# victorca25/traiNNer

Measured on AMD Instinct MI355X. Metric: HR images/sec (G+D step), ESRGAN x4 128->512, higher is better.
Workload: dtype f32 (bf16x3)

## Files before the change

include/trainner_hip.h:

```cpp
#ifndef TRAINNER_HIP_H
#define TRAINNER_HIP_H

#include <stdint.h>

#ifdef __cplusplus
extern "C" {
#endif

#define TNR_OK 0
#define TNR_EINVAL (-1)
#define TNR_ELAUNCH (-2)

enum { TNR_ACT_NONE = 0, TNR_ACT_LRELU = 1, TNR_ACT_RELU = 2 };

enum {
    TNR_CONV_3x3 = 0,
    TNR_CONV_3x3_UP2 = 1,
    TNR_CONV_4x4_S2 = 2,
    TNR_DGRAD_4x4_S2 = 3,
    TNR_CONV_1x1 = 4,
    TNR_CONV_3x3_C4 = 5,
    TNR_CONV_7x7_C4 = 6
};

// ... 13 lines not shown
#define TNR_MMA_BF16X3 2

typedef struct tnr_view {
    float *ptr;
    int32_t ctot;
    int32_t coff;
} tnr_view;

typedef struct tnr_conv_desc {
    tnr_view x;
    int32_t N, H, W;
    int32_t Cin;
    const float *wp;
    int32_t KinP, KoutP;
    tnr_view y;
    int32_t Ho, Wo, Cout;
    int32_t mode;
    const float *bias;
    int32_t act;
    float slope;
    float alpha;
    tnr_view r1; int32_t r1_ch; float beta1;
    tnr_view r2; float alpha2;
    tnr_view m;  int32_t m_lo, m_hi; float m_slope;
    float *ws; int64_t ws_bytes;
    int32_t mma;
    int32_t pad_mode;
    float noise_sigma; int32_t noise_pos; uint32_t noise_key0, noise_key1, noise_pix0;
    const void *wq; int64_t wq_bytes;
    int32_t wq_form;
    int32_t shuffle;
} tnr_conv_desc;

typedef struct tnr_wgrad_desc {
    tnr_view x; int32_t N, H, W; int32_t Cin;
    tnr_view g; int32_t Ho, Wo; int32_t Cout;
    int32_t mode;
    float *dw; int32_t cin_total, cin_begin;
    float *db;
    float alpha, beta;
    float *ws; int64_t ws_bytes;
    int32_t mma;
    int32_t pad_mode;
    float *dw2; int32_t cout_split, cin_total2;
    float *db2;
} tnr_wgrad_desc;

typedef struct tnr_pack_item {
    const float *w;
    float *wp;
    int32_t Cout, Cin, kh, kw;
    int32_t kind;
    int32_t KoutP, KinP;
    int64_t n_out;
} tnr_pack_item;

typedef struct tnr_dense_pack_item {
    const float *w[5];
    float *wp;
    int32_t nf, gc;
    int32_t t;
    int32_t KoutP, KinP;
    float scale5;
    int64_t n_out;
} tnr_dense_pack_item;

const char *tnr_last_error(void);
#define TNR_ABI_VERSION 3
int tnr_version(void);

int tnr_pack_dims(int32_t Cout, int32_t Cin, int32_t kh, int32_t kw, int32_t kind,
                  int32_t *KoutP, int32_t *KinP, int64_t *n_out);
int tnr_pack_weights(const tnr_pack_item *items_dev, int32_t n, int64_t max_out, void *stream);
int tnr_pack_dense_dims(int32_t nf, int32_t gc, int32_t t, int32_t *KoutP, int32_t *KinP, int64_t *n_out);
int tnr_pack_dense_dgrad(const tnr_dense_pack_item *items_dev, int32_t n, int64_t max_out, void *stream);
int tnr_conv_forward(const tnr_conv_desc *d, void *stream);
int tnr_gauss_mult(tnr_view dst, tnr_view src, int64_t pixels, int32_t C, float sigma, uint32_t key0, uint32_t key1, uint32_t pix0,
                   void *stream);
int64_t tnr_conv_workspace_bytes(const tnr_conv_desc *d);
int64_t tnr_conv_wq_bytes(const tnr_conv_desc *d);
int tnr_conv_wq_pack(const tnr_conv_desc *d, void *image, int64_t image_bytes, void *stream);
int64_t tnr_conv_wino_bytes(const tnr_conv_desc *d);
int tnr_conv_wino_pack(const tnr_conv_desc *d, void *image, int64_t image_bytes, void *stream);
int tnr_im2col(tnr_view x, int32_t N, int32_t H, int32_t W, int32_t C, int32_t k, int32_t stride, int32_t pad,
               int32_t Ho, int32_t Wo, float *out, void *stream);
#define TNR_CHAIN_MAX 6
int64_t tnr_conv_chain_workspace_bytes(const tnr_conv_desc *stage0);
int tnr_conv_chain(const tnr_conv_desc *stages, const int32_t *fresh_from, int32_t n, uint32_t *ws, int64_t ws_bytes,
                   uint32_t epoch, void *stream);
int64_t tnr_conv_sweep_image_bytes(const tnr_conv_desc *stages, int32_t n);
int tnr_conv_sweep_pack(const tnr_conv_desc *stages, int32_t n, void *image, int64_t image_bytes, void *stream);
typedef struct tnr_sweep_pack_item { int32_t units; int32_t reserved; uint64_t opaque[15]; } tnr_sweep_pack_item;
int tnr_conv_sweep_pack_item(const tnr_conv_desc *stages, int32_t n, void *image, int64_t image_bytes, tnr_sweep_pack_item *item);
int tnr_conv_sweep_pack_batch(const tnr_sweep_pack_item *items_dev, int32_t n, int32_t max_units, void *stream);
int tnr_conv_sweep(const tnr_conv_desc *stages, int32_t n, const void *image, uint32_t *ws, int64_t ws_bytes, uint32_t epoch,
                   void *stream);
int64_t tnr_conv_thin_pack_floats(int32_t reduce_channels);
int tnr_conv_thin_pack(const float *w_oihw, float *wp, int32_t Cout, int32_t Cin, int32_t dgrad, void *stream);
int tnr_conv_thin(tnr_view x, int32_t N, int32_t H, int32_t W, int32_t Cin, const float *wp, tnr_view y, int32_t Cout,
                  const float *bias, float alpha, void *stream);
int64_t tnr_conv_thin7_pack_floats(int32_t reduce_channels);
int tnr_conv_thin7_pack(const float *w_oihw, float *wp, int32_t Cout, int32_t Cin, int32_t dgrad, void *stream);
int tnr_conv_thin7(tnr_view x, int32_t N, int32_t H, int32_t W, int32_t Cin, const float *wp, tnr_view y, int32_t Ho, int32_t Wo,
                   int32_t Cout, int32_t pad, int32_t reflect, const float *bias, float alpha, void *stream);
int64_t tnr_wgrad_workspace_bytes(const tnr_wgrad_desc *d);
int64_t tnr_wgrad_thin_workspace_bytes(int32_t N, int32_t H, int32_t Cbig);
int tnr_wgrad_thin(tnr_view big, tnr_view small, int32_t N, int32_t H, int32_t W, int32_t Cbig, int32_t Csmall, int32_t flip,
                   float *dw, float *db, float alpha, float beta, float *ws, int64_t ws_bytes, void *stream);
int64_t tnr_wgrad_thin7_workspace_bytes(int32_t N, int32_t Hbig_grid, int32_t Cbig);
int tnr_wgrad_thin7(tnr_view big, int32_t N, int32_t H, int32_t W, int32_t rpad, tnr_view small, int32_t Hs, int32_t Ws, int32_t off,
                    int32_t Cbig, int32_t Csmall, int32_t flip, float *dw, float *db, float alpha, float beta, float *ws, int64_t ws_bytes,
                    void *stream);
int tnr_conv_wgrad(const tnr_wgrad_desc *d, void *stream);
#define TNR_WGRAD_GROUP_MAX 12
int tnr_conv_wgrad_group(const tnr_wgrad_desc *descs, int32_t n, void *stream);
int tnr_wgrad_tile_class(const tnr_wgrad_desc *d, int32_t group_jobs, int32_t x3_occ, int32_t out[12]);

int tnr_gconv_fwd(tnr_view x, int32_t N, int32_t H, int32_t W, int32_t Cin, const float *w, const float *bias, tnr_view y, int32_t Ho,
                  int32_t Wo, int32_t Cout, int32_t k, int32_t stride, int32_t pad, int32_t reflect, int32_t act, float slope, void *stream);
int tnr_gconv_dgrad(tnr_view g, int32_t N, int32_t H, int32_t W, int32_t Cin, const float *w, tnr_view gx, int32_t Ho, int32_t Wo,
                    int32_t Cout, int32_t k, int32_t stride, int32_t pad, int32_t reflect, void *stream);
int64_t tnr_gconv_wgrad_workspace_bytes(int32_t Cout, int32_t Cin, int32_t k);
int tnr_gconv_wgrad(tnr_view x, int32_t N, int32_t H, int32_t W, int32_t Cin, tnr_view g, int32_t Ho, int32_t Wo, int32_t Cout, int32_t k,
                    int32_t stride, int32_t pad, int32_t reflect, float *dw, float *db, float alpha, float beta, double *ws,
                    int64_t ws_bytes, void *stream);
int tnr_bias_grad(tnr_view g, int64_t pixels, int32_t C, float *db, float alpha, float beta, double *ws, int64_t ws_bytes, void *stream);
int tnr_pad2d(tnr_view x, tnr_view y, int32_t N, int32_t H, int32_t W, int32_t C, int32_t pad, int32_t mode, void *stream);
int tnr_unpad2d(tnr_view xp, tnr_view y, int32_t N, int32_t H, int32_t W, int32_t C, int32_t pad, int32_t mode, void *stream);
int tnr_window2d(tnr_view src, int32_t Hs, int32_t Ws, tnr_view dst, int32_t N, int32_t Hd, int32_t Wd, int32_t C, int32_t oy,
                 int32_t ox, int32_t acc, void *stream);
int tnr_tanh_fwd(const float *x, float *y, int64_t n, void *stream);
int tnr_tanh_bwd(const float *g, const float *y, float *gx, int64_t n, void *stream);
int tnr_gan_loss(const float *pred, int64_t n, int32_t type, float target, float *out, float *grad, void *stream);
int tnr_dp_unique_id(void *id128);
int tnr_dp_init(const void *id128, int32_t rank, int32_t world, void **comm);
int tnr_dp_allreduce_bucket(void *comm, float *buf, int64_t count, int32_t average, void *stream);
int tnr_dp_broadcast(void *comm, float *buf, int64_t count, int32_t root, void *stream);
int tnr_dp_comm_count(void *comm, int32_t *nranks);
int tnr_dp_finalize(void *comm);
int tnr_filter2d(const float *src, float *dst, const float *kernels21, int32_t N, int32_t C, int32_t H, int32_t W, void *stream);
int tnr_resize(const float *src, float *dst, int32_t NC, int32_t H, int32_t W, int32_t Ho, int32_t Wo, int32_t mode, void *stream);
int tnr_noise_gaussian(float *img, int32_t N, int32_t C, int32_t H, int32_t W, const float *sigma255, const int32_t *grey,
                       uint64_t seed, int32_t clip, void *stream);
int tnr_noise_poisson(float *img, int32_t N, int32_t C, int32_t H, int32_t W, const float *vals, const float *scale,
                      const int32_t *grey, uint64_t seed, int32_t clip, void *stream);
int64_t tnr_jpeg_workspace_bytes(int32_t N, int32_t H, int32_t W);
int tnr_jpeg_sim(float *img, int32_t N, int32_t H, int32_t W, const int32_t *quality, float *ws, int64_t ws_bytes, void *stream);
int tnr_feed_u8_to_tensor(const uint8_t *src, int32_t N, int32_t H, int32_t W, int32_t C, const int32_t *flags, int32_t any_rot,
                          float *dst, int32_t bgr2rgb, float data_range, int32_t normalize, void *stream);
int tnr_tensor2np_u8(const float *src, int32_t N, int32_t C, int32_t H, int32_t W, uint8_t *dst, int32_t rgb2bgr,
                     int32_t denormalize, void *stream);
int64_t tnr_metrics_workspace_bytes(int32_t N);
int tnr_psnr_ssim_u8(const uint8_t *a, const uint8_t *b, int32_t N, int32_t H, int32_t W, int32_t C, int32_t crop,
                     int32_t want_ssim, double *out, double *ws, int64_t ws_bytes, void *stream);
int tnr_lpips_stem_dims(int32_t H, int32_t W, int32_t crop, int32_t *Ho, int32_t *Wo);
int tnr_lpips_stem(const void *a, const void *b, int32_t src_kind, int32_t N, int32_t H, int32_t W, int32_t C, int32_t crop,
                   int32_t normalize, const float *shift, const float *scale, const float *w, const float *bias, tnr_view y,
                   void *stream);
int tnr_maxpool3s2_ceil_dims(int32_t H, int32_t W, int32_t *Ho, int32_t *Wo);
int tnr_maxpool3s2_ceil_fwd(tnr_view x, tnr_view y, int32_t N, int32_t H, int32_t W, int32_t C, void *stream);
int64_t tnr_lpips_workspace_bytes(int32_t N, int32_t L);
int tnr_lpips_head(tnr_view f0, tnr_view f1, int32_t N, int32_t H, int32_t W, int32_t C, const float *w, int32_t layer, int32_t L,
                   double *ws, int64_t ws_bytes, void *stream);
int tnr_lpips_finalize(int32_t N, int32_t L, const double *ws, int64_t ws_bytes, double *out, double *per_layer, void *stream);
int tnr_bilinear2x_fwd(tnr_view x, tnr_view y, int32_t N, int32_t H, int32_t W, int32_t C, void *stream);
int tnr_bilinear2x_bwd(tnr_view gy, tnr_view gx, tnr_view gz, tnr_view mask, float mslope, int32_t N, int32_t H, int32_t W,
// ... 151 lines not shown
```

trainner_amd/csrc/conv_wino.hip:

```cpp
#include <stddef.h>
#include <stdlib.h>
#include <type_traits>
#include <utility>
#include "conv_body.h"
#include "conv_epilogue.h"

namespace {

constexpr int WN_T = 16;
constexpr int WN_PT = WN_T / 2;
constexpr int WN_NP = WN_PT * WN_PT;
constexpr int WN_RAW_W = WN_T + 2;
constexpr int WN_RAW_PIX = WN_RAW_W * WN_RAW_W;
constexpr int WN_RAW_STRIDE = 24;
constexpr int WN_RAW_FLOATS = WN_RAW_PIX * WN_RAW_STRIDE;
constexpr int WN_ROW = TNR_X3_ROW;
constexpr int WN_VH_ROWS = 8 * WN_NP;
constexpr int WN_VH_FLOATS = WN_VH_ROWS * WN_ROW;
constexpr size_t WN_LDS_BYTES = (size_t)(2 * WN_VH_FLOATS + 2 * WN_RAW_FLOATS) * sizeof(float);
constexpr int WN_UNIT_FLOATS = 32 * WN_ROW;
constexpr int WN_STAGE_ITEMS = WN_RAW_PIX * 4;
constexpr int WN_STAGE_IT = (WN_STAGE_ITEMS / 2 + 255) / 256;
static_assert(WN_LDS_BYTES <= 160 * 1024, "one Winograd workgroup per CU");
static_assert(8 * 4 * 16 * 64 * sizeof(float) <= WN_LDS_BYTES, "the inverse transform's exchange fits the LDS");
// ... 523 lines not shown

        __syncthreads();
        raw_load(0, true);
        raw_store(0);
        raw_load(16, c.nck > 1);
        if (c.nck > 1) raw_store(1);
        __syncthreads();
        if (wh == 1) __syncthreads();
#pragma unroll 1
        for (int ck = 0; ck < c.nck; ++ck) {
            if (ck >= 1 && ck + 1 < c.nck) raw_store((ck + 1) & 1);
            transform(ck & 1);
            b_fetch(ck);
            __syncthreads();
            raw_load(16 * (ck + 2), ck + 2 < c.nck);
            multiply();
            __syncthreads();
        }
        if (wh == 0) __syncthreads();

        f32x16 pr_[2][2];
#pragma unroll
        for (int m = 0; m < 2; ++m) {
            if (wjp == 0) {
                pr_[0][m] = acc[0][m] + acc[1][m];
                pr_[1][m] = acc[1][m];
            } else {
                pr_[0][m] = acc[0][m];
                pr_[1][m] = -acc[0][m] - acc[1][m];
            }
        }
        float *xa = smem + (((wave & 3) | (wh << 2)) * 4) * (16 * 64);
        if (wjp == 1) {
#pragma unroll
            for (int l = 0; l < 2; ++l)
#pragma unroll
                for (int m = 0; m < 2; ++m)
#pragma unroll
                    for (int r = 0; r < 16; ++r) xa[((l * 2 + m) * 16 + r) * 64 + lane] = pr_[l][m][r];
        }
        __syncthreads();
        if (wjp == 0) {
#pragma unroll
            for (int l = 0; l < 2; ++l)
#pragma unroll
                for (int m = 0; m < 2; ++m)
#pragma unroll
                    for (int r = 0; r < 16; ++r) pr_[l][m][r] = l == 0 ? pr_[l][m][r] + xa[((l * 2 + m) * 16 + r) * 64 + lane]
                                                                       : pr_[l][m][r] + xa[((l * 2 + m) * 16 + r) * 64 + lane];
        }
        __syncthreads();
        float *xb = smem + ((wh * 4 + wn * 2 + wil) * 4) * (16 * 64);
        if (wjp == 0) {
#pragma unroll
            for (int l = 0; l < 2; ++l)
#pragma unroll
                for (int m = 0; m < 2; ++m)
#pragma unroll
                    for (int r = 0; r < 16; ++r) xb[((l * 2 + m) * 16 + r) * 64 + lane] = pr_[l][m][r];
        }
        __syncthreads();
        f32x16 keep[1][1];
        {
            const int k = wil, m = wh, l = wjp;
            auto slot = [&](int ip) __attribute__((always_inline)) {
                return smem + (((ip >> 1) * 4 + wn * 2 + (ip & 1)) * 4 + l * 2 + m) * (16 * 64) + lane;
            };
            const float *p0 = slot(k), *p1 = slot(k + 1), *p2 = slot(k + 2);
#pragma unroll
            for (int r = 0; r < 16; ++r) {
                const float x0 = p0[r * 64], x1 = p1[r * 64], x2 = p2[r * 64];
                keep[0][0][r] = k == 0 ? (x0 + x1) + x2 : (x0 - x1) - x2;
            }
        }
        conv_epilogue_dpp_map<TNR_CONV_3x3, WN_T, 1, 1, false, 1>(a, keep, cb * 2 + wn, n, ty0, tx0, 0, li, half, y_rs,
                                                                  [&](int, int row, int &rr, int &cc) __attribute__((always_inline)) {
                                                                      const int p = 32 * wh + row;
                                                                      rr = 2 * (p >> 3) + wil;
                                                                      cc = 2 * (p & 7) + wjp;
                                                                  });
    }
}

bool wino_ok(const tnr_conv_desc *d) {
    return d->mode == TNR_CONV_3x3 && d->mma == TNR_MMA_BF16X3 && (d->pad_mode == 0 || (d->pad_mode == 1 && d->H >= 2 && d->W >= 2)) &&
           (d->Cout % 64) == 0 && d->KoutP == d->Cout && d->Cin == d->KinP && (d->Cin % 16) == 0 && d->Cin >= 32 && d->Ho == d->H &&
           d->Wo == d->W && d->W >= 8 && d->H >= 8 && buffers_addressable(*d) &&
           (int64_t)(d->Cout / 64) * (d->Cin / 16) * 32 * WN_UNIT_FLOATS * (int64_t)sizeof(float) < (1LL << 31);
}

}

#ifdef WN_TIMELINE
extern "C" int tnr_debug_wino_timeline(unsigned long long *out16, int reset) {
    if (out16 != nullptr && hipMemcpyFromSymbol(out16, HIP_SYMBOL(wn_tl), sizeof(wn_tl)) != hipSuccess) return TNR_ELAUNCH;
    if (reset) {
        unsigned long long z[32] = {0};
        if (hipMemcpyToSymbol(HIP_SYMBOL(wn_tl), z, sizeof(z)) != hipSuccess) return TNR_ELAUNCH;
    }
    return TNR_OK;
}
#endif

extern "C" int64_t tnr_conv_wino_bytes(const tnr_conv_desc *d) {
    if (d == nullptr || !wino_ok(d)) return 0;
    return (int64_t)(d->Cout / 64) * (d->Cin / 16) * 32 * WN_UNIT_FLOATS * (int64_t)sizeof(float);
}

extern "C" int tnr_conv_wino_pack(const tnr_conv_desc *d, void *image, int64_t image_bytes, void *stream) {
    TNR_REQUIRE(d != nullptr && image != nullptr && d->wp != nullptr && wino_ok(d), "conv_wino_pack: the launch cannot run in the Winograd form");
    WinoPackK a;
    a.wp = d->wp; a.KinP = d->KinP; a.KoutP = d->KoutP; a.nck = d->Cin / 16; a.ncb = d->Cout / 64;
    a.units = a.ncb * a.nck * 32;
    TNR_REQUIRE((int64_t)a.units * WN_UNIT_FLOATS * (int64_t)sizeof(float) <= image_bytes, "conv_wino_pack: image buffer too small");
    a.out = static_cast<float *>(image);
    hipLaunchKernelGGL(wino_pack_kernel, dim3((unsigned)tnr_cdiv(a.units * 64, 256)), dim3(256), 0, (hipStream_t)stream, a);
    return tnr_check_launch("conv_wino_pack");
}

int tnr_launch_conv3x3_wino(const tnr_conv_desc *d, void *stream) {
    if (!wino_ok(d) || d->wq == nullptr || d->wq_bytes < tnr_conv_wino_bytes(d) || d->noise_pos < 0 || d->noise_pos > 2) return 1;
    static int cus = 0;
    if (const int rc = tnr_kernel_setup(&cus, "conv3x3_wino", {{conv3x3_wino_kernel, WN_LDS_BYTES}, {conv3x3_wino16_kernel, WN_LDS_BYTES}})) return rc;
    WinoK c;
    if (!stream_k_from_desc(c, *d, tnr_conv_wino_bytes(d), WN_T, WN_T, 1)) return 1;
    const int grid = c.tiles < cus ? c.tiles : cus;
    static const bool w16 = [] { const char *e = getenv("TNR_WINO_WAVES"); return e != nullptr && atoi(e) == 16; }();
    if (w16) {
        hipLaunchKernelGGL(conv3x3_wino16_kernel, dim3((unsigned)grid), dim3(1024), WN_LDS_BYTES, (hipStream_t)stream, c);
        return tnr_check_launch("conv3x3_wino16");
    }
    hipLaunchKernelGGL(conv3x3_wino_kernel, dim3((unsigned)grid), dim3(512), WN_LDS_BYTES, (hipStream_t)stream, c);
    return tnr_check_launch("conv3x3_wino");
}
```

trainner_amd/hip.py:

```python
import ctypes as C
import os

import torch

from . import build as _build

c_f = C.c_float
c_i = C.c_int32
c_l = C.c_int64
c_p = C.c_void_p

ACT_NONE, ACT_LRELU, ACT_RELU = 0, 1, 2
MMA_F32, MMA_BF16, MMA_BF16X3 = 0, 1, 2
CONV_3x3, CONV_3x3_UP2, CONV_4x4_S2, DGRAD_4x4_S2, CONV_1x1, CONV_3x3_C4, CONV_7x7_C4 = 0, 1, 2, 3, 4, 5, 6
PACK_FWD, PACK_DGRAD_3x3, PACK_FWD_S2D, PACK_DGRAD_S2, PACK_COL_FWD, PACK_COL_DGRAD3 = 0, 1, 2, 3, 4, 5
PACK_C4_FWD, PACK_C4_DGRAD3 = 6, 7
PACK_DENSE_DGRAD = 16


class CView(C.Structure):
    _fields_ = [("ptr", c_p), ("ctot", c_i), ("coff", c_i)]


class ConvDesc(C.Structure):
    _fields_ = [
        ("x", CView), ("N", c_i), ("H", c_i), ("W", c_i), ("Cin", c_i),
        ("wp", c_p), ("KinP", c_i), ("KoutP", c_i),
        ("y", CView), ("Ho", c_i), ("Wo", c_i), ("Cout", c_i),
        ("mode", c_i), ("bias", c_p), ("act", c_i), ("slope", c_f), ("alpha", c_f),
        ("r1", CView), ("r1_ch", c_i), ("beta1", c_f),
        ("r2", CView), ("alpha2", c_f),
        ("m", CView), ("m_lo", c_i), ("m_hi", c_i), ("m_slope", c_f),
        ("ws", c_p), ("ws_bytes", c_l), ("mma", c_i), ("pad_mode", c_i),
        ("noise_sigma", c_f), ("noise_pos", c_i), ("noise_key0", C.c_uint32), ("noise_key1", C.c_uint32), ("noise_pix0", C.c_uint32),
        ("wq", c_p), ("wq_bytes", c_l), ("wq_form", c_i), ("shuffle", c_i),
    ]


class WgradDesc(C.Structure):
    _fields_ = [
        ("x", CView), ("N", c_i), ("H", c_i), ("W", c_i), ("Cin", c_i),
        ("g", CView), ("Ho", c_i), ("Wo", c_i), ("Cout", c_i),
        ("mode", c_i),
        ("dw", c_p), ("cin_total", c_i), ("cin_begin", c_i),
        ("db", c_p), ("alpha", c_f), ("beta", c_f),
        ("ws", c_p), ("ws_bytes", c_l), ("mma", c_i), ("pad_mode", c_i),
        ("dw2", c_p), ("cout_split", c_i), ("cin_total2", c_i), ("db2", c_p),
    ]


class SweepPackItem(C.Structure):
    _fields_ = [("units", c_i), ("reserved", c_i), ("opaque", C.c_uint64 * 15)]


class PackItem(C.Structure):
    _fields_ = [("w", c_p), ("wp", c_p), ("Cout", c_i), ("Cin", c_i), ("kh", c_i), ("kw", c_i),
                ("kind", c_i), ("KoutP", c_i), ("KinP", c_i), ("n_out", c_l)]


class DensePackItem(C.Structure):
    _fields_ = [("w", c_p * 5), ("wp", c_p), ("nf", c_i), ("gc", c_i), ("t", c_i), ("KoutP", c_i), ("KinP", c_i),
                ("scale5", c_f), ("n_out", c_l)]


_SIGS = {
    "tnr_last_error": (C.c_char_p, []),
    "tnr_version": (c_i, []),
    "tnr_pack_dims": (c_i, [c_i, c_i, c_i, c_i, c_i, C.POINTER(c_i), C.POINTER(c_i), C.POINTER(c_l)]),
    "tnr_pack_weights": (c_i, [c_p, c_i, c_l, c_p]),
    "tnr_pack_dense_dims": (c_i, [c_i, c_i, c_i, C.POINTER(c_i), C.POINTER(c_i), C.POINTER(c_l)]),
    "tnr_pack_dense_dgrad": (c_i, [c_p, c_i, c_l, c_p]),
    "tnr_conv_forward": (c_i, [C.POINTER(ConvDesc), c_p]),
    "tnr_conv_workspace_bytes": (c_l, [C.POINTER(ConvDesc)]),
    "tnr_conv_wq_bytes": (c_l, [C.POINTER(ConvDesc)]),
    "tnr_conv_wq_pack": (c_i, [C.POINTER(ConvDesc), c_p, c_l, c_p]),
    "tnr_conv_wino_bytes": (c_l, [C.POINTER(ConvDesc)]),
    "tnr_conv_wino_pack": (c_i, [C.POINTER(ConvDesc), c_p, c_l, c_p]),
    "tnr_gauss_mult": (c_i, [CView, CView, c_l, c_i, c_f, C.c_uint32, C.c_uint32, C.c_uint32, c_p]),
    "tnr_im2col": (c_i, [CView, c_i, c_i, c_i, c_i, c_i, c_i, c_i, c_i, c_i, c_p, c_p]),
    "tnr_conv_chain_workspace_bytes": (c_l, [C.POINTER(ConvDesc)]),
    "tnr_conv_chain": (c_i, [C.POINTER(ConvDesc), C.POINTER(C.c_int32), c_i, c_p, c_l, C.c_uint32, c_p]),
    "tnr_conv_sweep_image_bytes": (c_l, [C.POINTER(ConvDesc), c_i]),
    "tnr_conv_sweep_pack_item": (c_i, [C.POINTER(ConvDesc), c_i, c_p, c_l, C.POINTER(SweepPackItem)]),
    "tnr_conv_sweep_pack_batch": (c_i, [c_p, c_i, c_i, c_p]),
    "tnr_conv_sweep_pack": (c_i, [C.POINTER(ConvDesc), c_i, c_p, c_l, c_p]),
    "tnr_conv_sweep": (c_i, [C.POINTER(ConvDesc), c_i, c_p, c_p, c_l, C.c_uint32, c_p]),
    "tnr_conv_thin_pack_floats": (c_l, [c_i]),
    "tnr_conv_thin_pack": (c_i, [c_p, c_p, c_i, c_i, c_i, c_p]),
    "tnr_conv_thin": (c_i, [CView, c_i, c_i, c_i, c_i, c_p, CView, c_i, c_p, c_f, c_p]),
    "tnr_wgrad_workspace_bytes": (c_l, [C.POINTER(WgradDesc)]),
    "tnr_conv_thin7_pack_floats": (c_l, [c_i]),
    "tnr_conv_thin7_pack": (c_i, [c_p, c_p, c_i, c_i, c_i, c_p]),
    "tnr_conv_thin7": (c_i, [CView, c_i, c_i, c_i, c_i, c_p, CView, c_i, c_i, c_i, c_i, c_i, c_p, c_f, c_p]),
    "tnr_wgrad_thin7_workspace_bytes": (c_l, [c_i, c_i, c_i]),
    "tnr_wgrad_thin7": (c_i, [CView, c_i, c_i, c_i, c_i, CView, c_i, c_i, c_i, c_i, c_i, c_i, c_p, c_p, c_f, c_f, c_p, c_l, c_p]),
    "tnr_wgrad_thin_workspace_bytes": (c_l, [c_i, c_i, c_i]),
    "tnr_wgrad_thin": (c_i, [CView, CView, c_i, c_i, c_i, c_i, c_i, c_i, c_p, c_p, c_f, c_f, c_p, c_l, c_p]),
    "tnr_conv_wgrad": (c_i, [C.POINTER(WgradDesc), c_p]),
    "tnr_conv_wgrad_group": (c_i, [C.POINTER(WgradDesc), c_i, c_p]),
    "tnr_wgrad_tile_class": (c_i, [C.POINTER(WgradDesc), c_i, c_i, C.POINTER(c_i * 12)]),
    "tnr_nchw_to_nhwc": (c_i, [c_p, c_i, c_i, c_i, c_i, CView, c_i, c_p, c_p, c_p]),
    "tnr_nhwc_to_nchw": (c_i, [CView, c_i, c_i, c_i, c_i, c_p, c_p, c_i, c_p]),
    "tnr_upsample2x_bwd": (c_i, [CView, CView, c_i, c_i, c_i, c_i, CView, c_f, c_p]),
    "tnr_depth_to_space": (c_i, [CView, CView, c_i, c_i, c_i, c_i, c_p]),
    "tnr_space_to_depth_bwd": (c_i, [CView, CView, c_i, c_i, c_i, c_i, CView, c_f, c_p]),
    "tnr_maxpool2_fwd": (c_i, [CView, CView, c_i, c_i, c_i, c_i, c_p]),
    "tnr_maxpool2_bwd": (c_i, [CView, CView, CView, c_i, c_i, c_i, c_i, c_p]),
    "tnr_gconv_fwd": (c_i, [CView, c_i, c_i, c_i, c_i, c_p, c_p, CView, c_i, c_i, c_i, c_i, c_i, c_i, c_i, c_i, c_f, c_p]),
    "tnr_gconv_dgrad": (c_i, [CView, c_i, c_i, c_i, c_i, c_p, CView, c_i, c_i, c_i, c_i, c_i, c_i, c_i, c_p]),
    "tnr_gconv_wgrad_workspace_bytes": (c_l, [c_i, c_i, c_i]),
    "tnr_gconv_wgrad": (c_i, [CView, c_i, c_i, c_i, c_i, CView, c_i, c_i, c_i, c_i, c_i, c_i, c_i, c_p, c_p, c_f, c_f, c_p, c_l, c_p]),
    "tnr_bias_grad": (c_i, [CView, c_l, c_i, c_p, c_f, c_f, c_p, c_l, c_p]),
    "tnr_pad2d": (c_i, [CView, CView, c_i, c_i, c_i, c_i, c_i, c_i, c_p]),
    "tnr_unpad2d": (c_i, [CView, CView, c_i, c_i, c_i, c_i, c_i, c_i, c_p]),
    "tnr_window2d": (c_i, [CView, c_i, c_i, CView, c_i, c_i, c_i, c_i, c_i, c_i, c_i, c_p]),
    "tnr_tanh_fwd": (c_i, [c_p, c_p, c_l, c_p]),
    "tnr_tanh_bwd": (c_i, [c_p, c_p, c_p, c_l, c_p]),
    "tnr_gan_loss": (c_i, [c_p, c_l, c_i, c_f, c_p, c_p, c_p]),
    "tnr_dp_unique_id": (c_i, [c_p]),
    "tnr_dp_init": (c_i, [c_p, c_i, c_i, C.POINTER(c_p)]),
    "tnr_dp_allreduce_bucket": (c_i, [c_p, c_p, c_l, c_i, c_p]),
    "tnr_dp_broadcast": (c_i, [c_p, c_p, c_l, c_i, c_p]),
    "tnr_dp_comm_count": (c_i, [c_p, C.POINTER(c_i)]),
    "tnr_dp_finalize": (c_i, [c_p]),
    "tnr_filter2d": (c_i, [c_p, c_p, c_p, c_i, c_i, c_i, c_i, c_p]),
    "tnr_resize": (c_i, [c_p, c_p, c_i, c_i, c_i, c_i, c_i, c_i, c_p]),
    "tnr_noise_gaussian": (c_i, [c_p, c_i, c_i, c_i, c_i, c_p, c_p, C.c_uint64, c_i, c_p]),
    "tnr_noise_poisson": (c_i, [c_p, c_i, c_i, c_i, c_i, c_p, c_p, c_p, C.c_uint64, c_i, c_p]),
    "tnr_jpeg_workspace_bytes": (c_l, [c_i, c_i, c_i]),
    "tnr_jpeg_sim": (c_i, [c_p, c_i, c_i, c_i, c_p, c_p, c_l, c_p]),
    "tnr_feed_u8_to_tensor": (c_i, [c_p, c_i, c_i, c_i, c_i, c_p, c_i, c_p, c_i, c_f, c_i, c_p]),
    "tnr_tensor2np_u8": (c_i, [c_p, c_i, c_i, c_i, c_i, c_p, c_i, c_i, c_p]),
    "tnr_metrics_workspace_bytes": (c_l, [c_i]),
    "tnr_psnr_ssim_u8": (c_i, [c_p, c_p, c_i, c_i, c_i, c_i, c_i, c_i, c_p, c_p, c_l, c_p]),
    "tnr_lpips_stem_dims": (c_i, [c_i, c_i, c_i, C.POINTER(c_i), C.POINTER(c_i)]),
    "tnr_lpips_stem": (c_i, [c_p, c_p, c_i, c_i, c_i, c_i, c_i, c_i, c_i, c_p, c_p, c_p, c_p, CView, c_p]),
    "tnr_maxpool3s2_ceil_dims": (c_i, [c_i, c_i, C.POINTER(c_i), C.POINTER(c_i)]),
    "tnr_maxpool3s2_ceil_fwd": (c_i, [CView, CView, c_i, c_i, c_i, c_i, c_p]),
    "tnr_lpips_workspace_bytes": (c_l, [c_i, c_i]),
    "tnr_lpips_head": (c_i, [CView, CView, c_i, c_i, c_i, c_i, c_p, c_i, c_i, c_p, c_l, c_p]),
    "tnr_lpips_finalize": (c_i, [c_i, c_i, c_p, c_l, c_p, c_p, c_p]),
    "tnr_bilinear2x_fwd": (c_i, [CView, CView, c_i, c_i, c_i, c_i, c_p]),
    "tnr_bilinear2x_bwd": (c_i, [CView, CView, CView, CView, c_f, c_i, c_i, c_i, c_i, c_p]),
    "tnr_add2": (c_i, [CView, CView, CView, c_l, c_i, c_p]),
    "tnr_mask_copy": (c_i, [CView, CView, CView, c_l, c_i, c_f, c_p]),
    "tnr_axpby": (c_i, [CView, CView, c_l, c_i, c_f, c_f, c_p]),
    "tnr_mask_mul": (c_i, [CView, CView, c_l, c_i, c_f, c_p]),
    "tnr_fill": (c_i, [c_p, c_l, c_f, c_p]),
    "tnr_bn_workspace_bytes": (c_l, [c_i]),
    "tnr_bn_train_fwd": (c_i, [CView, CView, c_l, c_i, c_p, c_p, c_p, c_p, c_p, c_f, c_f, c_p, c_p, c_i, c_f, c_p, c_p]),
    "tnr_bn_train_fwd_stats": (c_i, [CView, CView, c_l, c_i, c_p, c_p, c_p, c_p, c_p, c_f, c_f, c_p, c_p, c_p, c_i, c_f, c_p, c_p]),
    "tnr_bn_replay_running": (c_i, [c_p, c_p, c_p, c_p, c_i, c_f, c_p]),
    "tnr_bn_train_bwd": (c_i, [CView, CView, CView, CView, c_l, c_i, c_p, c_p, c_p, c_f, c_p, c_p, c_f, c_p, c_p]),
    "tnr_bn_train_bwd_z": (c_i, [CView, CView, CView, c_l, c_i, c_p, c_p, c_p, c_p, c_f, c_p, c_p, c_f, c_p, c_p]),
    "tnr_instnorm_workspace_bytes": (c_l, [c_i, c_i]),
    "tnr_instnorm_fwd": (c_i, [CView, CView, c_i, c_l, c_i, c_f, c_p, c_p, c_i, c_f, c_p, c_p]),
    "tnr_instnorm_bwd": (c_i, [CView, CView, CView, CView, c_i, c_l, c_i, c_p, c_p, c_f, c_p, c_p]),
    "tnr_linear_fwd": (c_i, [c_p, c_p, c_p, c_p, c_i, c_i, c_i, c_i, c_f, c_p]),
    "tnr_linear_bwd": (c_i, [c_p, c_p, c_p, c_p, c_f, c_p, c_p, c_p, c_i, c_i, c_i, c_f, c_p, c_p]),
    "tnr_reduce_workspace_bytes": (c_l, []),
# ... 122 lines not shown
```

Before: 73.32.

## Add 4-wave Winograd conv kernel and select it for deep channel reductions

Adds a 256-thread (4-wave) variant of the Winograd 3x3 conv kernel in which each wave computes all four transform positions for its output slice, with a software-pipelined loop that interleaves MFMA, input transforms, raw loads and weight fetches. By default it is chosen when the channel-chunk count is at least 12, otherwise the 8-wave kernel is kept, and an API/env override is added. The goal is to cut cross-wave synchronisation and LDS traffic per MFMA for long reductions, at the cost of fewer waves per CU to hide latency and higher register pressure.

```diff
diff --git a/include/trainner_hip.h b/include/trainner_hip.h
--- a/include/trainner_hip.h
+++ b/include/trainner_hip.h
@@ -119,6 +119,7 @@
 int tnr_conv_wq_pack(const tnr_conv_desc *d, void *image, int64_t image_bytes, void *stream);
 int64_t tnr_conv_wino_bytes(const tnr_conv_desc *d);
 int tnr_conv_wino_pack(const tnr_conv_desc *d, void *image, int64_t image_bytes, void *stream);
+int tnr_conv_wino_waves(int32_t set);
 int tnr_im2col(tnr_view x, int32_t N, int32_t H, int32_t W, int32_t C, int32_t k, int32_t stride, int32_t pad,
                int32_t Ho, int32_t Wo, float *out, void *stream);
 #define TNR_CHAIN_MAX 6
diff --git a/trainner_amd/csrc/conv_wino.hip b/trainner_amd/csrc/conv_wino.hip
--- a/trainner_amd/csrc/conv_wino.hip
+++ b/trainner_amd/csrc/conv_wino.hip
@@ -629,6 +629,246 @@
     }
 }
 
+constexpr int W4_STAGE_IT = (WN_STAGE_ITEMS + 255) / 256;
+constexpr int W4_ITEM_RAW = 4 * WN_RAW_W * WN_RAW_STRIDE;
+constexpr int W4_ITEM_V = 16 * WN_ROW;
+constexpr int W4_XCH = 8 * 16 * 64;
+static_assert(4 * W4_XCH * sizeof(float) <= WN_LDS_BYTES, "the inverse transform's exchange fits the LDS");
+static_assert((3 * W4_ITEM_RAW + 4 * WN_RAW_STRIDE) * sizeof(float) < 65536, "an item's raw reads address by immediate offsets");
+
+__global__ void __launch_bounds__(256, 1) conv3x3_wino4_kernel(const WinoK c) {
+    extern __shared__ __attribute__((aligned(16))) float smem[];
+    float *s_v = smem;
+    float *s_raw = smem + 2 * WN_VH_FLOATS;
+    const int tid = threadIdx.x;
+    const int wave = __builtin_amdgcn_readfirstlane(tid >> 6), lane = tid & 63, li = lane & 31, half = lane >> 5;
+    const ConvK &a = c.a;
+    const __amdgpu_buffer_rsrc_t x_rs =
+        __builtin_amdgcn_make_buffer_rsrc(const_cast<float *>(a.x), 0, (int)((unsigned)a.N * a.H * a.W * a.x_ct * 4u), 0x00020000);
+    const __amdgpu_buffer_rsrc_t w_rs = __builtin_amdgcn_make_buffer_rsrc(const_cast<float *>(c.wq), 0, c.wq_bytes, 0x00020000);
+    const __amdgpu_buffer_rsrc_t y_rs =
+        __builtin_amdgcn_make_buffer_rsrc(a.y, 0, (int)((unsigned)a.N * a.Ho * a.Wo * a.y_ct * 4u), 0x00020000);
+
+    const int l4 = lane >> 2, tq = lane & 3;
+    const int pa = wave == 0 ? 0 : (wave == 2 ? 2 : 1), pb = wave == 0 ? 2 : (wave == 1 ? 2 : (wave == 2 ? 1 : 3));
+    const float sgn = wave == 1 ? 1.f : -1.f;
+    const int raw_a = ((2 * (l4 >> 3) + pa) * WN_RAW_W + 2 * (l4 & 7)) * WN_RAW_STRIDE + 4 * tq;
+    const int raw_b = ((2 * (l4 >> 3) + pb) * WN_RAW_W + 2 * (l4 & 7)) * WN_RAW_STRIDE + 4 * tq;
+    static_assert(TNR_X3_SWZ < 4, "the swizzle bit must not depend on the transform position, the item or the M-tile");
+    constexpr int XL_STRIDE = WN_NP * WN_ROW;
+    float *v_dst = s_v + (wave * 4 * WN_NP + l4) * WN_ROW + 4 * ((tq >> 1) ^ ((l4 >> TNR_X3_SWZ) & 1)) + 2 * (tq & 1);
+    const float *a_src = s_v + (wave * 4 * WN_NP + li) * WN_ROW + 4 * (half ^ ((li >> TNR_X3_SWZ) & 1));
+
+    for (int tile = blockIdx.x; tile < c.tiles; tile += gridDim.x) {
+        const int cb = tile % c.ncb;
+        int rest = tile / c.ncb;
+        const int tx = rest % c.tiles_x;
+        rest /= c.tiles_x;
+        const int ty = rest % c.tiles_y, n = rest / c.tiles_y;
+        const int ty0 = ty * WN_T, tx0 = tx * WN_T;
+        int tid_t = wave * 64 + (int)__builtin_amdgcn_mbcnt_hi(~0u, __builtin_amdgcn_mbcnt_lo(~0u, 0u));
+        asm volatile("" : "+v"(tid_t));
+        int in_off[W4_STAGE_IT];
+#pragma unroll
+        for (int it = 0; it < W4_STAGE_IT; ++it) {
+            const int i = tid_t + it * 256, pix = i >> 2, q = i & 3;
+            const int pr = pix / WN_RAW_W, pc = pix - pr * WN_RAW_W;
+            int Y = ty0 + pr - 1, X = tx0 + pc - 1;
+            if (a.reflect) {
+                Y = Y == -1 ? 1 : (Y == a.H ? a.H - 2 : Y);
+                X = X == -1 ? 1 : (X == a.W ? a.W - 2 : X);
+            }
+            const bool in = (i < WN_STAGE_ITEMS) & (Y >= 0) & (Y < a.H) & (X >= 0) & (X < a.W);
+            in_off[it] = in ? (((n * a.H + Y) * a.W + X) * a.x_ct + a.x_co + q * 4) : -1;
+        }
+        const bool last_mine = tid_t < WN_STAGE_ITEMS - (W4_STAGE_IT - 1) * 256;
+        const int r_dst0 = (tid_t >> 2) * WN_RAW_STRIDE + 4 * (tid_t & 3);
+        static_assert(W4_STAGE_IT == 6, "two batches of three items");
+        f32x4 rin[3];
+        auto raw_load1 = [&](f32x4 &dst, auto itc, int ch, bool valid) __attribute__((always_inline)) {
+            constexpr int it = decltype(itc)::value;
+            const unsigned bo = (valid && in_off[it] >= 0) ? (unsigned)(in_off[it] + ch) * 4u : 0xfffffff0u;
+            dst = __builtin_bit_cast(f32x4, __builtin_amdgcn_raw_buffer_load_b128(x_rs, (int)bo, 0, 0));
+        };
+        auto raw_store1 = [&](const f32x4 &src, auto itc, int buf) __attribute__((always_inline)) {
+            constexpr int it = decltype(itc)::value;
+            if (it + 1 < W4_STAGE_IT || last_mine)
+                *reinterpret_cast<f32x4 *>(s_raw + buf * WN_RAW_FLOATS + r_dst0 + it * 64 * WN_RAW_STRIDE) = src;
+        };
+
+        tnr_bf16x8 fbr[4][2][3];
+        const int bq0 = ((cb * 2 * 4 + wave) * c.nck) * 4, bq_nt = 4 * c.nck * 4;
+        auto b_fetch1 = [&](int ck, auto jc, auto ntc, int sp) __attribute__((always_inline)) {
+            constexpr int j = decltype(jc)::value, nt = decltype(ntc)::value;
+            const int u = bq0 + nt * bq_nt + ck * 4 + j;
+            fbr[j][nt][sp] = __builtin_bit_cast(tnr_bf16x8, __builtin_amdgcn_raw_buffer_load_b128(w_rs, lane * 16, (u * 3 + sp) * 1024, 0));
+        };
+
+        f32x4 rr[4][2], e[4], sv, sr, bk;
+        unsigned sh0 = 0, sh1 = 0, sm0 = 0, sm1 = 0;
+        auto cvt2 = [](float x0, float x1) __attribute__((always_inline)) {
+            const tnr_f32x2 p = {x0, x1};
+            return __builtin_bit_cast(unsigned, __builtin_convertvector(p, tnr_bf16x2));
+        };
+        auto xf_step = [&](auto kc, auto tc, const float *raw) __attribute__((always_inline)) {
+            constexpr int K = decltype(kc)::value, T = decltype(tc)::value;
+            if constexpr (T < 2) {
+                constexpr int QA = T == 0 ? 1 : 0, QB = T == 0 ? 2 : 3;
+                rr[QA][0] = *reinterpret_cast<const f32x4 *>(raw + raw_a + K * W4_ITEM_RAW + QA * WN_RAW_STRIDE);
+                rr[QA][1] = *reinterpret_cast<const f32x4 *>(raw + raw_b + K * W4_ITEM_RAW + QA * WN_RAW_STRIDE);
+                rr[QB][0] = *reinterpret_cast<const f32x4 *>(raw + raw_a + K * W4_ITEM_RAW + QB * WN_RAW_STRIDE);
+                rr[QB][1] = *reinterpret_cast<const f32x4 *>(raw + raw_b + K * W4_ITEM_RAW + QB * WN_RAW_STRIDE);
+            } else if constexpr (T < 4) {
+                constexpr int QA = T == 2 ? 1 : 0, QB = T == 2 ? 2 : 3;
+#pragma unroll
+                for (int x = 0; x < 4; ++x) {
+                    e[QA][x] = __builtin_fmaf(rr[QA][1][x], sgn, rr[QA][0][x]);
+                    e[QB][x] = __builtin_fmaf(rr[QB][1][x], sgn, rr[QB][0][x]);
+                }
+            } else {
+                constexpr int J = (T - 4) / 5, S = (T - 4) % 5;
+                if constexpr (S == 0) {
+                    sv = J == 0 ? e[0] - e[2] : (J == 1 ? e[1] + e[2] : (J == 2 ? e[2] - e[1] : e[1] - e[3]));
+                    sh0 = cvt2(sv[0], sv[1]);
+                    sh1 = cvt2(sv[2], sv[3]);
+                } else if constexpr (S == 1) {
+                    bk = f32x4{__builtin_bit_cast(float, sh0 << 16), __builtin_bit_cast(float, sh0 & 0xffff0000u),
+                               __builtin_bit_cast(float, sh1 << 16), __builtin_bit_cast(float, sh1 & 0xffff0000u)};
+                    sr[0] = sv[0] - bk[0];
+                    sr[1] = sv[1] - bk[1];
+                } else if constexpr (S == 2) {
+                    sr[2] = sv[2] - bk[2];
+                    sr[3] = sv[3] - bk[3];
+                    sm0 = cvt2(sr[0], sr[1]);
+                    sm1 = cvt2(sr[2], sr[3]);
+                    bk[0] = __builtin_bit_cast(float, sm0 << 16);
+                    bk[1] = __builtin_bit_cast(float, sm0 & 0xffff0000u);
+                } else if constexpr (S == 3) {
+                    bk[2] = __builtin_bit_cast(float, sm1 << 16);
+                    bk[3] = __builtin_bit_cast(float, sm1 & 0xffff0000u);
+                    sr = sr - bk;
+                } else {
+                    const unsigned l0 = cvt2(sr[0], sr[1]), l1 = cvt2(sr[2], sr[3]);
+                    float *d = v_dst + J * XL_STRIDE + K * W4_ITEM_V;
+                    *reinterpret_cast<tnr_f32x2 *>(d) = tnr_f32x2{__builtin_bit_cast(float, sh0), __builtin_bit_cast(float, sh1)};
+                    *reinterpret_cast<tnr_f32x2 *>(d + 8) = tnr_f32x2{__builtin_bit_cast(float, sm0), __builtin_bit_cast(float, sm1)};
+                    *reinterpret_cast<tnr_f32x2 *>(d + 16) = tnr_f32x2{__builtin_bit_cast(float, l0), __builtin_bit_cast(float, l1)};
+                }
+            }
+        };
+
+        f32x16 acc[4][2][2];
+        __syncthreads();
+        {
+            f32x4 rin0[W4_STAGE_IT], rin1[W4_STAGE_IT];
+            wn_static_for<0, W4_STAGE_IT>([&](auto itc) __attribute__((always_inline)) { raw_load1(rin0[decltype(itc)::value], itc, 0, true); });
+            wn_static_for<0, W4_STAGE_IT>([&](auto itc) __attribute__((always_inline)) { raw_load1(rin1[decltype(itc)::value], itc, 16, c.nck > 1); });
+            wn_static_for<0, 4>([&](auto jc) __attribute__((always_inline)) {
+                wn_static_for<0, 2>([&](auto ntc) __attribute__((always_inline)) {
+                    if constexpr (decltype(jc)::value != 3 || decltype(ntc)::value != 1) {
+#pragma unroll
+                        for (int sp = 0; sp < 3; ++sp) b_fetch1(0, jc, ntc, sp);
+                    }
+                });
+            });
+            __builtin_amdgcn_sched_barrier(0);
+#pragma unroll
+            for (int j = 0; j < 4; ++j)
+#pragma unroll
+                for (int m = 0; m < 2; ++m)
+#pragma unroll
+                    for (int nt = 0; nt < 2; ++nt) {
+#pragma unroll
+                        for (int r = 0; r < 16; ++r) acc[j][m][nt][r] = 0.f;
+                        asm volatile("" : "+a"(acc[j][m][nt]));
+                    }
+            __builtin_amdgcn_sched_barrier(0);
+            wn_static_for<0, W4_STAGE_IT>([&](auto itc) __attribute__((always_inline)) { raw_store1(rin0[decltype(itc)::value], itc, 0); });
+            wn_static_for<0, W4_STAGE_IT>([&](auto itc) __attribute__((always_inline)) { raw_store1(rin1[decltype(itc)::value], itc, 1); });
+        }
+        __syncthreads();
+        wn_static_for<0, 48>([&](auto sc) __attribute__((always_inline)) {
+            constexpr int s = decltype(sc)::value;
+            xf_step(std::integral_constant<int, s / 24>{}, std::integral_constant<int, s % 24>{}, s_raw);
+        });
+        wn_static_for<0, 6>([&](auto sc) __attribute__((always_inline)) { xf_step(std::integral_constant<int, 2>{}, sc, s_raw); });
+        tnr_bf16x8 fa[2][3];
+#pragma unroll
+        for (int sp = 0; sp < 3; ++sp) fa[0][sp] = *reinterpret_cast<const tnr_bf16x8 *>(a_src + 8 * sp);
+
+        constexpr int TA[6] = {0, 2, 1, 0, 1, 0}, TB[6] = {2, 0, 1, 1, 0, 0};
+#pragma unroll 1
+        for (int ck = 0; ck < c.nck; ++ck) {
+            const bool has_next = ck + 1 < c.nck;
+            const int ck_next = has_next ? ck + 1 : ck;
+            const float *raw_cur = s_raw + (ck & 1) * WN_RAW_FLOATS, *raw_nxt = s_raw + ((ck + 1) & 1) * WN_RAW_FLOATS;
+            wn_static_for<0, 96>([&](auto gc) __attribute__((always_inline)) {
+                constexpr int gg = decltype(gc)::value, m = gg / 48, g = gg % 48, j = g / 12, nt = (g / 6) % 2, p = g % 6, U = 4 * m + j;
+                acc[j][m][nt] = __builtin_amdgcn_mfma_f32_32x32x16_bf16(fa[U & 1][TA[p]], fbr[j][nt][TB[p]], acc[j][m][nt], 0, 0, 0);
+                if constexpr (g % 12 >= 6 && g % 12 < 9) {
+                    constexpr int U1 = (U + 1) % 8, m1 = U1 / 4, j1 = U1 % 4, sp = g % 12 - 6;
+                    fa[U1 & 1][sp] = *reinterpret_cast<const tnr_bf16x8 *>(a_src + j1 * XL_STRIDE + m1 * 32 * WN_ROW + 8 * sp);
+                }
+                if constexpr (m == 0 && g < 3) b_fetch1(ck, std::integral_constant<int, 3>{}, std::integral_constant<int, 1>{}, g);
+                if constexpr (m == 1 && g >= 6 && (g - 6) % 6 < 3)
+                    b_fetch1(ck_next, std::integral_constant<int, (g - 6) / 12>{}, std::integral_constant<int, ((g - 6) / 6) % 2>{}, (g - 6) % 6);
+                if constexpr (g >= 3 && g < 6) raw_load1(rin[g % 3], std::integral_constant<int, 3 * m + g % 3>{}, 16 * (ck + 2), ck + 2 < c.nck);
+                if constexpr (g >= 45) {
+                    if (ck + 2 < c.nck) raw_store1(rin[g % 3], std::integral_constant<int, 3 * m + g % 3>{}, ck & 1);
+                }
+                if constexpr (m == 0 && g == 41) asm volatile("s_waitcnt lgkmcnt(0)\n\ts_barrier" ::: "memory");
+                {
+                    constexpr int s = g >= 42 ? g - 42 : g + 6, T = s % 24;
+                    constexpr int K = (g >= 42 ? (m == 0 ? 0 : 2) : (m == 0 ? 2 : 0)) + s / 24;
+                    xf_step(std::integral_constant<int, K>{}, std::integral_constant<int, T>{}, (m == 0 && g < 42) ? raw_cur : raw_nxt);
+                }
+                __builtin_amdgcn_sched_barrier(0);
+            });
+        }
+
+        asm volatile("s_waitcnt lgkmcnt(0)\n\ts_barrier" ::: "memory");
+        int lane_t = (int)__builtin_amdgcn_mbcnt_hi(~0u, __builtin_amdgcn_mbcnt_lo(~0u, 0u));
+        asm volatile("" : "+v"(lane_t));
+        {
+            float *xch = smem + wave * W4_XCH;
+#pragma unroll
+            for (int l = 0; l < 2; ++l)
+#pragma unroll
+                for (int m = 0; m < 2; ++m)
+#pragma unroll
+                    for (int nt = 0; nt < 2; ++nt) {
+                        const f32x16 q = l == 0 ? (acc[0][m][nt] + acc[1][m][nt]) + acc[2][m][nt] : (acc[1][m][nt] - acc[2][m][nt]) - acc[3][m][nt];
+#pragma unroll
+                        for (int r = 0; r < 16; ++r) xch[(((l * 2 + m) * 2 + nt) * 16 + r) * 64 + lane_t] = q[r];
+                        __builtin_amdgcn_sched_barrier(0);
+                    }
+        }
+        __syncthreads();
+        const int k = wave & 1, m = wave >> 1;
+        const int li_t = lane_t & 31, half_t = lane_t >> 5;
+#pragma unroll 1
+        for (int nt = 0; nt < 2; ++nt) {
+            f32x16 keep[2][1];
+#pragma unroll
+            for (int l = 0; l < 2; ++l) {
+                const float *p0 = smem + k * W4_XCH + (((l * 2 + m) * 2 + nt) * 16) * 64 + lane_t, *p1 = p0 + W4_XCH, *p2 = p1 + W4_XCH;
+#pragma unroll
+                for (int r = 0; r < 16; ++r) {
+                    const float x0 = p0[r * 64], x1 = p1[r * 64], x2 = p2[r * 64];
+                    keep[l][0][r] = k == 0 ? (x0 + x1) + x2 : (x0 - x1) - x2;
+                }
+            }
+            conv_epilogue_dpp_map<TNR_CONV_3x3, WN_T, 1, 2, false, 1>(a, keep, cb * 2 + nt, n, ty0, tx0, 0, li_t, half_t, y_rs,
+                                                                      [&](int mi, int row, int &rr_, int &cc_) __attribute__((always_inline)) {
+                                                                          const int pp = 32 * m + row;
+                                                                          rr_ = 2 * (pp >> 3) + k;
+                                                                          cc_ = 2 * (pp & 7) + mi;
+                                                                      });
+            __builtin_amdgcn_sched_barrier(0);
+        }
+    }
+}
+
 bool wino_ok(const tnr_conv_desc *d) {
     return d->mode == TNR_CONV_3x3 && d->mma == TNR_MMA_BF16X3 && (d->pad_mode == 0 || (d->pad_mode == 1 && d->H >= 2 && d->W >= 2)) &&
            (d->Cout % 64) == 0 && d->KoutP == d->Cout && d->Cin == d->KinP && (d->Cin % 16) == 0 && d->Cin >= 32 && d->Ho == d->H &&
@@ -636,6 +876,28 @@
            (int64_t)(d->Cout / 64) * (d->Cin / 16) * 32 * WN_UNIT_FLOATS * (int64_t)sizeof(float) < (1LL << 31);
 }
 
+#ifndef WN4_MIN_NCK
+#define WN4_MIN_NCK 12
+#endif
+int wino_waves_override = 0;
+int wino_waves_choice() {
+    static const int env = [] {
+        const char *e = getenv("TNR_WINO_WAVES");
+        const int v = e != nullptr ? atoi(e) : 0;
+        return (v == 4 || v == 8 || v == 16) ? v : 0;
+    }();
+    return wino_waves_override != 0 ? wino_waves_override : env;
+}
+int wino_waves(int nck) {
+    const int v = wino_waves_choice();
+    return v != 0 ? v : (nck >= WN4_MIN_NCK ? 4 : 8);
+}
+
+}
+
+extern "C" int tnr_conv_wino_waves(int set) {
+    if (set == 4 || set == 8 || set == 16 || set == 0) wino_waves_override = set;
+    return wino_waves_choice();
 }
 
 #ifdef WN_TIMELINE
@@ -668,15 +930,20 @@
 int tnr_launch_conv3x3_wino(const tnr_conv_desc *d, void *stream) {
     if (!wino_ok(d) || d->wq == nullptr || d->wq_bytes < tnr_conv_wino_bytes(d) || d->noise_pos < 0 || d->noise_pos > 2) return 1;
     static int cus = 0;
-    if (const int rc = tnr_kernel_setup(&cus, "conv3x3_wino", {{conv3x3_wino_kernel, WN_LDS_BYTES}, {conv3x3_wino16_kernel, WN_LDS_BYTES}})) return rc;
+    if (const int rc = tnr_kernel_setup(&cus, "conv3x3_wino", {{conv3x3_wino_kernel, WN_LDS_BYTES}, {conv3x3_wino16_kernel, WN_LDS_BYTES},
+                                                                {conv3x3_wino4_kernel, WN_LDS_BYTES}})) return rc;
     WinoK c;
     if (!stream_k_from_desc(c, *d, tnr_conv_wino_bytes(d), WN_T, WN_T, 1)) return 1;
     const int grid = c.tiles < cus ? c.tiles : cus;
-    static const bool w16 = [] { const char *e = getenv("TNR_WINO_WAVES"); return e != nullptr && atoi(e) == 16; }();
-    if (w16) {
+    const int waves = wino_waves(c.nck);
+    if (waves == 16) {
         hipLaunchKernelGGL(conv3x3_wino16_kernel, dim3((unsigned)grid), dim3(1024), WN_LDS_BYTES, (hipStream_t)stream, c);
         return tnr_check_launch("conv3x3_wino16");
     }
+    if (waves == 4) {
+        hipLaunchKernelGGL(conv3x3_wino4_kernel, dim3((unsigned)grid), dim3(256), WN_LDS_BYTES, (hipStream_t)stream, c);
+        return tnr_check_launch("conv3x3_wino4");
+    }
     hipLaunchKernelGGL(conv3x3_wino_kernel, dim3((unsigned)grid), dim3(512), WN_LDS_BYTES, (hipStream_t)stream, c);
     return tnr_check_launch("conv3x3_wino");
 }
diff --git a/trainner_amd/hip.py b/trainner_amd/hip.py
--- a/trainner_amd/hip.py
+++ b/trainner_amd/hip.py
@@ -76,6 +76,7 @@
     "tnr_conv_wq_pack": (c_i, [C.POINTER(ConvDesc), c_p, c_l, c_p]),
     "tnr_conv_wino_bytes": (c_l, [C.POINTER(ConvDesc)]),
     "tnr_conv_wino_pack": (c_i, [C.POINTER(ConvDesc), c_p, c_l, c_p]),
+    "tnr_conv_wino_waves": (c_i, [c_i]),
     "tnr_gauss_mult": (c_i, [CView, CView, c_l, c_i, c_f, C.c_uint32, C.c_uint32, C.c_uint32, c_p]),
     "tnr_im2col": (c_i, [CView, c_i, c_i, c_i, c_i, c_i, c_i, c_i, c_i, c_i, c_p, c_p]),
     "tnr_conv_chain_workspace_bytes": (c_l, [C.POINTER(ConvDesc)]),
```

Measured after the change: 74.02 (median of 6 runs). No clear change (+0.9%).
